# QCLovers/PyTDSCF

Hardware: NVIDIA B200
Metric: tdvp_sweeps_per_sec (higher is better)
Workload: dtype complex128

## Files before the change

pytdscf_b200/csrc/api.cu:

```cuda
#include <cstring>

#include "contract.cuh"

namespace tdvp {

int krylov_expm_exec(Handle* h, int kind, double scale_re, double scale_im, double thresh, int n_warmup,
                     int conserve_norm, const tdvp_heff_term* hterms, const tdvp_keff_term* kterms, int nterms,
                     int Dl, int d, int Dr, c128* psi, int* niter);
int lanczos_eigvec_exec(Handle* h, const tdvp_heff_term* hterms, int nterms, int Dl, int d, int Dr, c128* psi, int root,
                        double thresh, int* niter);
int inner_exec(Handle* h, long long n, const c128* bra, const c128* ket, int conj, c128* host_out);
int qr_shift_exec(Handle* h, int gauge, int Dl, int d, int Dr, const c128* psi, c128* site, c128* sigma);
int absorb_exec(Handle* h, int gauge, int Dl, int d, int Dr, int k, const c128* sigma, const c128* site, c128* out);
int qr_configure(Handle* h);
int svd_configure(Handle* h);

void set_error(Handle* h, const std::string& msg) {
  if (h) h->err = msg;
}

int cuda_fail(Handle* h, cudaError_t e, const char* what, const char* file, int line) {
  char buf[512];
  snprintf(buf, sizeof(buf), "CUDA error %d (%s) in %s at %s:%d", (int)e, cudaGetErrorString(e), what, file, line);
  set_error(h, buf);
  return (int)e > 0 ? (int)e : 1;
}

int ws_reserve(Handle* h, size_t bytes) {
  h->ws_top = 0;
  if (bytes <= h->ws_bytes) return 0;
  size_t want = bytes + bytes / 4 + (size_t(1) << 20);
  TDVP_CUDA(h, cudaStreamSynchronize(h->stream));
  if (h->side) TDVP_CUDA(h, cudaStreamSynchronize(h->side));
  if (h->ws) TDVP_CUDA(h, cudaFree(h->ws));
  h->ws = nullptr;
  h->ws_bytes = 0;
  void* p = nullptr;
  TDVP_CUDA(h, cudaMalloc(&p, want));
  h->ws = (unsigned char*)p;
  h->ws_bytes = want;
  return 0;
}

int ws_grow_preserve(Handle* h, size_t bytes) {
  if (bytes <= h->ws_bytes) return 0;
  void* p = nullptr;
  TDVP_CUDA(h, cudaMalloc(&p, bytes));
  if (h->ws) {
    cudaError_t e = cudaMemcpyAsync(p, h->ws, h->ws_top, cudaMemcpyDeviceToDevice, h->stream);
    if (e == cudaSuccess) e = cudaStreamSynchronize(h->stream);
    if (e != cudaSuccess) { cudaFree(p); return cuda_fail(h, e, "ws_grow_preserve copy", __FILE__, __LINE__); }
    TDVP_CUDA(h, cudaFree(h->ws));
  }
  h->ws = (unsigned char*)p;
  h->ws_bytes = bytes;
  return 0;
}

void* ws_alloc(Handle* h, size_t bytes) {
  const size_t b = align256(bytes);
  if (h->ws_top + b > h->ws_bytes) return nullptr;
  void* p = h->ws + h->ws_top;
  h->ws_top += b;
  return p;
}

}

using namespace tdvp;

struct tdvp_handle_s : public tdvp::Handle {};

#define H_CHECK(h)            \
  if (!(h)) return TDVP_ERR_ARG; \
  (h)->err.clear();

extern "C" {

int tdvp_abi_version(void) { return 2; }

unsigned long long tdvp_launch_count(void) { return tdvp::launch_count(); }

int tdvp_create(int device, void* cuda_stream, tdvp_handle_t* out) {
  if (!out) return TDVP_ERR_ARG;
  *out = nullptr;
  int ndev = 0;
  cudaError_t e = cudaGetDeviceCount(&ndev);
  if (e != cudaSuccess || ndev <= 0) return e != cudaSuccess ? (int)e : (int)cudaErrorNoDevice;
  if (device < 0 || device >= ndev) return TDVP_ERR_ARG;
  if ((e = cudaSetDevice(device)) != cudaSuccess) return (int)e;
  tdvp_handle_s* h = new tdvp_handle_s();
  h->device = device;
  h->stream = (cudaStream_t)cuda_stream;
  if ((e = cudaMalloc((void**)&h->d_scal, 4096 * sizeof(double))) != cudaSuccess) { delete h; return (int)e; }
  if ((e = cudaMallocHost((void**)&h->h_scal, 4096 * sizeof(double))) != cudaSuccess) { delete h; return (int)e; }
  if ((e = cudaMalloc((void**)&h->d_partial, 1024 * 64 * sizeof(double))) != cudaSuccess) { delete h; return (int)e; }
  if ((e = cudaMalloc((void**)&h->d_counter, 16 * sizeof(unsigned int))) != cudaSuccess) { delete h; return (int)e; }
  if ((e = cudaMalloc((void**)&h->d_splitk, tdvp::SPLITK_SCRATCH_ELEMS * sizeof(c128))) != cudaSuccess) { delete h; return (int)e; }
  if ((e = cudaMalloc((void**)&h->d_partial_side, 1024 * 64 * sizeof(double))) != cudaSuccess ||
      (e = cudaMalloc((void**)&h->d_counter_side, 16 * sizeof(unsigned int))) != cudaSuccess ||
      (e = cudaStreamCreateWithFlags(&h->side, cudaStreamNonBlocking)) != cudaSuccess ||
      (e = cudaEventCreateWithFlags(&h->ev_main, cudaEventDisableTiming)) != cudaSuccess ||
      (e = cudaEventCreateWithFlags(&h->ev_side, cudaEventDisableTiming)) != cudaSuccess) { tdvp_destroy(h); return (int)e; }
  cudaMemsetAsync(h->d_counter, 0, 16 * sizeof(unsigned int), h->stream);
  cudaMemsetAsync(h->d_counter_side, 0, 16 * sizeof(unsigned int), h->stream);
  cudaMemsetAsync(h->d_scal, 0, 4096 * sizeof(double), h->stream);
  memset(h->h_scal, 0, 4096 * sizeof(double));
  cudaDeviceGetAttribute(&h->num_sms, cudaDevAttrMultiProcessorCount, device);
  h->gemm.stream = h->stream;
  h->gemm.scratch = h->d_splitk;
  h->gemm.scratch_elems = tdvp::SPLITK_SCRATCH_ELEMS;
  h->gemm.num_sms = h->num_sms;
  h->gemm.sk_slots = h->num_sms;
  if ((e = cudaMalloc((void**)&h->gemm.sk_ws, sizeof(c128) * tdvp::STREAMK_TILE_ELEMS * (size_t)h->num_sms)) != cudaSuccess ||
      (e = cudaMalloc((void**)&h->gemm.sk_flags, sizeof(int) * (size_t)h->num_sms)) != cudaSuccess) { tdvp_destroy(h); return (int)e; }
  cudaMemsetAsync(h->gemm.sk_flags, 0, sizeof(int) * (size_t)h->num_sms, h->stream);
  int rc = 0;
  if ((e = tdvp::zgemm_configure_device(h->gemm)) != cudaSuccess) rc = (int)e;
  if (!rc) rc = tdvp::qr_configure(h);
  if (!rc) rc = tdvp::svd_configure(h);
  if (rc) { tdvp_destroy(h); return rc; }
  *out = h;
  return 0;
}

int tdvp_set_gemm_config(tdvp_handle_t h, int tile_cfg, int splitk, int c_stream) {
  if (!h || tile_cfg < 0 || tile_cfg > 5 || splitk < 0 || splitk > 16 || c_stream < 0 || c_stream > 2) return TDVP_ERR_ARG;
  h->gemm.force_cfg = tile_cfg;
  h->gemm.force_splitk = splitk;
  h->gemm.force_cstream = c_stream;
  return 0;
}

int tdvp_destroy(tdvp_handle_t h) {
  if (!h) return 0;
  cudaSetDevice(h->device);
  cudaStreamSynchronize(h->stream);
  if (h->ws) cudaFree(h->ws);
  if (h->d_scal) cudaFree(h->d_scal);
  if (h->h_scal) cudaFreeHost(h->h_scal);
  if (h->d_partial) cudaFree(h->d_partial);
  if (h->d_counter) cudaFree(h->d_counter);
  if (h->d_splitk) cudaFree(h->d_splitk);
  if (h->side) { cudaStreamSynchronize(h->side); cudaStreamDestroy(h->side); }
  if (h->ev_main) cudaEventDestroy(h->ev_main);
  if (h->ev_side) cudaEventDestroy(h->ev_side);
  if (h->d_partial_side) cudaFree(h->d_partial_side);
  if (h->d_counter_side) cudaFree(h->d_counter_side);
  if (h->gemm.sk_ws) cudaFree(h->gemm.sk_ws);
  if (h->gemm.sk_flags) cudaFree(h->gemm.sk_flags);
  delete h;
  return 0;
}

const char* tdvp_last_error(tdvp_handle_t h) { return h ? h->err.c_str() : "null handle"; }

int tdvp_get_stats(tdvp_handle_t h, unsigned long long* solves, unsigned long long* matvecs, double* flops) {
  if (!h) return TDVP_ERR_ARG;
  if (solves) *solves = h->krylov_solves;
  if (matvecs) *matvecs = h->krylov_matvecs;
  if (flops) *flops = h->heff_flops;
  return 0;
}

int tdvp_reset_stats(tdvp_handle_t h) {
  if (!h) return TDVP_ERR_ARG;
  h->krylov_solves = 0;
  h->krylov_matvecs = 0;
  h->heff_flops = 0.0;
  return 0;
}

int tdvp_gemm_profile(int enable, int reset, double* ms, double* flops, unsigned long long* launches) {
  tdvp::prof_collect(false);
  tdvp::prof_gemm_totals(ms, flops, launches);
  if (reset) tdvp::prof_collect(true);
  tdvp::prof_enable(enable != 0);
  return 0;
}

size_t tdvp_profile_json(char* out, size_t cap) {
  tdvp::prof_collect(false);
  return tdvp::prof_json(out, cap);
}

int tdvp_heff_apply(tdvp_handle_t h, const tdvp_heff_term* terms, int nterms, int Dl, int d, int Dr,
                    const tdvp_c128* psi, tdvp_c128* out) {
  H_CHECK(h);
  if (!terms || !psi || !out || Dl <= 0 || d <= 0 || Dr <= 0) { set_error(h, "heff_apply: bad argument"); return TDVP_ERR_ARG; }
  if (psi == out) { set_error(h, "heff_apply: out must not alias psi"); return TDVP_ERR_ARG; }
  TDVP_TRY(ws_reserve(h, sizeof(c128) * heff_ws_elems(terms, nterms, Dl, d, Dr)));
  return heff_apply_exec(h, terms, nterms, Dl, d, Dr, (const c128*)psi, (c128*)out);
}

int tdvp_keff_apply(tdvp_handle_t h, const tdvp_keff_term* terms, int nterms, int Dl, int Dr, const tdvp_c128* sigma,
                    tdvp_c128* out) {
  H_CHECK(h);
  if (!terms || !sigma || !out || Dl <= 0 || Dr <= 0) { set_error(h, "keff_apply: bad argument"); return TDVP_ERR_ARG; }
  if (sigma == out) { set_error(h, "keff_apply: out must not alias sigma"); return TDVP_ERR_ARG; }
  TDVP_TRY(ws_reserve(h, sizeof(c128) * keff_ws_elems(terms, nterms, Dl, Dr)));
  return keff_apply_exec(h, terms, nterms, Dl, Dr, (const c128*)sigma, (c128*)out);
}

int tdvp_env_update(tdvp_handle_t h, int gauge, int Dl, int d, int Dr, const tdvp_c128* bra, const tdvp_c128* ket,
                    const tdvp_c128* E, int w_in, const tdvp_c128* W, int w_kind, int w_out, tdvp_c128* out,
                    int accumulate) {
  H_CHECK(h);
  if (!bra || !ket || !out || Dl <= 0 || d <= 0 || Dr <= 0 || w_in <= 0 || w_out <= 0) { set_error(h, "env_update: bad argument"); return TDVP_ERR_ARG; }
  TDVP_TRY(ws_reserve(h, sizeof(c128) * env_ws_elems(Dl, d, Dr, w_in, w_out)));
  return env_update_exec(h, gauge, Dl, d, Dr, (const c128*)bra, (const c128*)ket, (const c128*)E, w_in, (const c128*)W,
                         w_kind, w_out, (c128*)out, accumulate != 0);
}

int tdvp_set_krylov_size(tdvp_handle_t hh, long long size) {
  Handle* h = reinterpret_cast<Handle*>(hh);
  if (!h || size < 0) return TDVP_ERR_ARG;
  h->krylov_size_override = size;
  return 0;
}

int tdvp_krylov_expm(tdvp_handle_t h, int kind, double scale_re, double scale_im, double thresh, int n_warmup,
                     int conserve_norm, const tdvp_heff_term* hterms, const tdvp_keff_term* kterms, int nterms, int Dl,
                     int d, int Dr, tdvp_c128* psi_inout, int* niter) {
  H_CHECK(h);
  if (!psi_inout || nterms <= 0 || Dl <= 0 || Dr <= 0 || (hterms && d <= 0)) { set_error(h, "krylov_expm: bad argument"); return TDVP_ERR_ARG; }
  return krylov_expm_exec(h, kind, scale_re, scale_im, thresh, n_warmup, conserve_norm, hterms, kterms, nterms, Dl, d, Dr,
                          (c128*)psi_inout, niter);
}

int tdvp_lanczos_eigvec(tdvp_handle_t h, const tdvp_heff_term* hterms, int nterms, int Dl, int d, int Dr,
                        tdvp_c128* psi_inout, int root, double thresh, int* niter) {
  H_CHECK(h);
  if (!hterms || !psi_inout || nterms <= 0 || Dl <= 0 || d <= 0 || Dr <= 0) { set_error(h, "lanczos_eigvec: bad argument"); return TDVP_ERR_ARG; }
  return lanczos_eigvec_exec(h, hterms, nterms, Dl, d, Dr, (c128*)psi_inout, root, thresh, niter);
}

int tdvp_qr_shift(tdvp_handle_t h, int gauge, int Dl, int d, int Dr, const tdvp_c128* psi, tdvp_c128* site,
                  tdvp_c128* sigma) {
  H_CHECK(h);
  if (!psi || !site || !sigma || Dl <= 0 || d <= 0 || Dr <= 0) { set_error(h, "qr_shift: bad argument"); return TDVP_ERR_ARG; }
  return qr_shift_exec(h, gauge, Dl, d, Dr, (const c128*)psi, (c128*)site, (c128*)sigma);
}

int tdvp_absorb(tdvp_handle_t h, int gauge, int Dl, int d, int Dr, int k, const tdvp_c128* sigma, const tdvp_c128* site,
                tdvp_c128* out) {
  H_CHECK(h);
  if (!sigma || !site || !out || Dl <= 0 || d <= 0 || Dr <= 0 || k <= 0) { set_error(h, "absorb: bad argument"); return TDVP_ERR_ARG; }
  return absorb_exec(h, gauge, Dl, d, Dr, k, (const c128*)sigma, (const c128*)site, (c128*)out);
}

int tdvp_inner(tdvp_handle_t h, long long n, const tdvp_c128* bra, const tdvp_c128* ket, int conj, tdvp_c128* host_out) {
  H_CHECK(h);
  if (!bra || !ket || !host_out || n <= 0) { set_error(h, "inner: bad argument"); return TDVP_ERR_ARG; }
  return inner_exec(h, n, (const c128*)bra, (const c128*)ket, conj, (c128*)host_out);
}

int tdvp_overlap_site(tdvp_handle_t h, int Dlb, int Dlk, int d, int Drb, int Drk, const tdvp_c128* bra,
                      const tdvp_c128* ket, const tdvp_c128* block, int conj_bra, tdvp_c128* out) {
  H_CHECK(h);
  if (!bra || !ket || !block || !out) { set_error(h, "overlap_site: bad argument"); return TDVP_ERR_ARG; }
  TDVP_TRY(ws_reserve(h, sizeof(c128) * ((size_t)Dlb * d * Drk + 64)));
  return overlap_site_exec(h, Dlb, Dlk, d, Drb, Drk, (const c128*)bra, (const c128*)ket, (const c128*)block, conj_bra,
                           (c128*)out);
}

int tdvp_zgemm(tdvp_handle_t h, int transA, int transB, int M, int N, int K, double alpha_re, double alpha_im,
               const tdvp_c128* A, int lda, const tdvp_c128* B, int ldb, double beta_re, double beta_im, tdvp_c128* C,
               int ldc) {
  H_CHECK(h);
  if (!A || !B || !C || M < 0 || N < 0 || K < 0 || transA < 0 || transA > 2 || transB < 0 || transB > 2) {
    set_error(h, "zgemm: bad argument");
    return TDVP_ERR_ARG;
  }
  GemmDesc g = gemm_rowmajor(M, N, K, (const c128*)A, lda, transA != 0, transA == 2, (const c128*)B, ldb, transB != 0,
                             (c128*)C, ldc, c128{alpha_re, alpha_im}, c128{beta_re, beta_im});
  g.b_conj = transB == 2 ? 1 : 0;
  return gemm(h, g);
}

}
```

pytdscf_b200/csrc/build.py:

```python
from __future__ import annotations

import hashlib
import os
import subprocess
import sys

HERE = os.path.dirname(os.path.abspath(__file__))
PKG = os.path.dirname(HERE)
SOURCES = ["api.cu", "zgemm.cu", "zgemm_tma.cu", "contract.cu", "krylov.cu", "qr.cu", "svd.cu"]
HEADERS = ["common.cuh", "handle.cuh", "contract.cuh", "zgemm_plan.h", os.path.join("..", "..", "include", "tdvp_b200.h")]
OUT = os.path.join(PKG, "libtdvp_b200.so")
NVCC_FLAGS = [
    "-gencode", "arch=compute_100a,code=sm_100a",
    "-O3", "-lineinfo", "-std=c++17",
    "-Xcompiler", "-fPIC",
]


def _digest() -> str:
    h = hashlib.sha256()
    for f in SOURCES + HEADERS:
        p = os.path.join(HERE, f)
        if os.path.exists(p):
            h.update(open(p, "rb").read())
    h.update(" ".join(NVCC_FLAGS).encode())
    return h.hexdigest()


def build(force: bool = False, verbose: bool = True) -> str:
    stamp = OUT + ".sha256"
    dig = _digest()
    if not force and os.path.exists(OUT) and os.path.exists(stamp) and open(stamp).read().strip() == dig:
        return OUT
    nvcc = os.environ.get("NVCC", "nvcc")
    objs = []
    os.makedirs(os.path.join(HERE, "_obj"), exist_ok=True)
    procs = []
    for src in SOURCES:
        sp = os.path.join(HERE, src)
        if not os.path.exists(sp):
            continue
        obj = os.path.join(HERE, "_obj", src.replace(".cu", ".o"))
        objs.append(obj)
        cmd = [nvcc, *NVCC_FLAGS, "-c", sp, "-o", obj]
        if verbose:
            print("[build]", " ".join(cmd), flush=True)
        procs.append((src, subprocess.Popen(cmd, stdout=subprocess.PIPE, stderr=subprocess.STDOUT, text=True)))
    failed = False
    for src, p in procs:
        out, _ = p.communicate()
        if p.returncode != 0:
            failed = True
            print(f"[build] {src} FAILED:\n{out}", file=sys.stderr)
        elif out.strip() and verbose:
            print(out)
    if failed:
        raise RuntimeError("nvcc failed")
    cmd = [nvcc, "-gencode", "arch=compute_100a,code=sm_100a", "-shared", "-o", OUT, *objs, "-lcudart"]
    if verbose:
        print("[build]", " ".join(cmd), flush=True)
    subprocess.check_call(cmd)
    with open(stamp, "w") as f:
        f.write(dig)
    return OUT


if __name__ == "__main__":
    print(build(force="--force" in sys.argv))
```

pytdscf_b200/csrc/handle.cuh:

```cuda
#pragma once
#include "common.cuh"

#include <vector>

namespace tdvp {

struct Handle {
  int device = 0;
  cudaStream_t stream = nullptr;
  std::string err;
  unsigned char* ws = nullptr;
  size_t ws_bytes = 0;
  size_t ws_top = 0;
  double* d_scal = nullptr;
  double* h_scal = nullptr;
  double* d_partial = nullptr;
  unsigned int* d_counter = nullptr;
  c128* d_splitk = nullptr;
  cudaStream_t side = nullptr;
  cudaEvent_t ev_main = nullptr, ev_side = nullptr;
  double* d_partial_side = nullptr;
  unsigned int* d_counter_side = nullptr;
  GemmCtx gemm;
  int num_sms = 148;
  int qr_max_cluster = 0;
  int svd_max_blocks = 0;
  int svd_blocked_max_blocks = 0;
  unsigned long long krylov_matvecs = 0;
  unsigned long long krylov_solves = 0;
  long long krylov_size_override = 0;
  double heff_flops = 0.0;
};

int ws_reserve(Handle* h, size_t bytes);
int ws_grow_preserve(Handle* h, size_t bytes);
void* ws_alloc(Handle* h, size_t bytes);
inline void ws_reset(Handle* h) { h->ws_top = 0; }
inline size_t align256(size_t b) { return (b + 255) & ~size_t(255); }

}
```

pytdscf_b200/csrc/qr.cu:

```cuda
#include <cooperative_groups.h>

#include "contract.cuh"

namespace cg = cooperative_groups;

namespace tdvp {

namespace {

constexpr int NB = 32;
constexpr int SLAB_ROWS = 256;
constexpr int PT = 256;
constexpr int PTY = PT / 32;

struct PanelArgs {
  c128* A; int lda; int m; int n; int j0; int jb;
  double* tau;
  c128* Vall;
  c128* Tall;
  double* gpart;
  double* zpart;
  int rows_per_cta;
  c128* gslab;
  int dbg;
};

__device__ __forceinline__ double dlapy3(double x, double y, double z) {
  const double w = fmax(fabs(x), fmax(fabs(y), fabs(z)));
  if (w == 0.0) return 0.0;
  const double a = x / w, b = y / w, c = z / w;
  return w * sqrt(a * a + b * b + c * c);
}

__global__ void __launch_bounds__(PT, 1) k_qr_panel(PanelArgs p) {
  extern __shared__ __align__(16) unsigned char smraw[];
  c128* S = p.gslab ? p.gslab + (size_t)blockIdx.x * p.rows_per_cta * NB : reinterpret_cast<c128*>(smraw);
  __shared__ c128 red[PTY][NB];
  __shared__ c128 gtot[NB];
  __shared__ c128 rowc[NB];
  __shared__ c128 wv[NB];
  __shared__ double s_tau[2], s_scal[2], s_beta;
  cg::grid_group grid = cg::this_grid();
  const int tx = threadIdx.x, ty = threadIdx.y;
  const int G = gridDim.x, b = blockIdx.x;
  const int jb = p.jb, j0 = p.j0;
  const int r0 = j0 + b * p.rows_per_cta;
  int nrow = p.m - r0;
  if (nrow > p.rows_per_cta) nrow = p.rows_per_cta;
  if (nrow < 0) nrow = 0;

  for (int i = ty; i < nrow; i += PTY) {
    if (tx < jb) S[i * NB + tx] = p.A[(long long)(r0 + i) * p.lda + j0 + tx];
    else S[i * NB + tx] = {0.0, 0.0};
  }
  __syncthreads();

  for (int c = 0; c < jb; ++c) {
    const int grow = j0 + c;
    double* gp = p.gpart + (size_t)(c & 1) * G * (4 * NB);
    c128 acc = {0.0, 0.0};
    if (tx >= c && tx < jb) {
      for (int i = ty; i < nrow; i += PTY) {
        if (r0 + i > grow) {
          const c128 x = S[i * NB + c], y = S[i * NB + tx];
          acc.x += x.x * y.x + x.y * y.y;
          acc.y += x.x * y.y - x.y * y.x;
        }
      }
    }
    red[ty][tx] = acc;
    __syncthreads();
    if (ty == 0) {
      c128 t = {0.0, 0.0};
#pragma unroll
      for (int q = 0; q < PTY; ++q) { t.x += red[q][tx].x; t.y += red[q][tx].y; }
      gp[(size_t)b * (4 * NB) + 2 * tx] = t.x;
      gp[(size_t)b * (4 * NB) + 2 * tx + 1] = t.y;
      if (grow >= r0 && grow < r0 + nrow) {
        const c128 v = S[(grow - r0) * NB + tx];
        gp[2 * NB + 2 * tx] = v.x;
        gp[2 * NB + 2 * tx + 1] = v.y;
      }
    }
    __threadfence();
    if (G > 1) grid.sync(); else __syncthreads();
    if (ty == 0) {
      c128 t = {0.0, 0.0};
      for (int q = 0; q < G; ++q) {
        t.x += __ldcg(&gp[(size_t)q * (4 * NB) + 2 * tx]);
        t.y += __ldcg(&gp[(size_t)q * (4 * NB) + 2 * tx + 1]);
      }
      gtot[tx] = t;
      rowc[tx] = {__ldcg(&gp[2 * NB + 2 * tx]), __ldcg(&gp[2 * NB + 2 * tx + 1])};
    }
    __syncthreads();
    if (tx == 0 && ty == 0) {
      const bool tiny_tail = gtot[c].x < 1.0e-200;
      const double xnorm = tiny_tail ? 0.0 : sqrt(gtot[c].x);
      const double alphr = rowc[c].x, alphi = rowc[c].y;
      if (xnorm == 0.0 && alphi == 0.0) {
        s_tau[0] = 0.0; s_tau[1] = 0.0; s_scal[0] = 1.0; s_scal[1] = 0.0; s_beta = alphr;
      } else if (tiny_tail) {
        const double beta = (alphr >= 0.0) ? -hypot(alphr, alphi) : hypot(alphr, alphi);
        s_tau[0] = (beta - alphr) / beta;
        s_tau[1] = -alphi / beta;
        s_scal[0] = 0.0; s_scal[1] = 0.0;
        s_beta = beta;
      } else {
        double beta = dlapy3(alphr, alphi, xnorm);
        beta = (alphr >= 0.0) ? -beta : beta;
        s_tau[0] = (beta - alphr) / beta;
        s_tau[1] = -alphi / beta;
        const double dr = alphr - beta, di = alphi;
        const double den = dr * dr + di * di;
        s_scal[0] = dr / den; s_scal[1] = -di / den;
        s_beta = beta;
      }
      if (b == 0) { p.tau[2 * (j0 + c)] = s_tau[0]; p.tau[2 * (j0 + c) + 1] = s_tau[1]; }
    }
    __syncthreads();
    const c128 tau = {s_tau[0], s_tau[1]};
    const c128 sc = {s_scal[0], s_scal[1]};
    const bool trivial = (tau.x == 0.0 && tau.y == 0.0);
    if (ty == 0 && tx > c && tx < jb) {
      const c128 cs = {sc.x, -sc.y};
      wv[tx] = cadd(rowc[tx], cmul(cs, gtot[tx]));
    }
    __syncthreads();
    if (!trivial) {
      const c128 ctau = {tau.x, -tau.y};
      for (int i = ty; i < nrow; i += PTY) {
        const int gr = r0 + i;
        if (gr < grow) continue;
        c128 v;
        if (gr == grow) v = {1.0, 0.0};
        else v = cmul(S[i * NB + c], sc);
        if (tx > c && tx < jb) {
          const c128 f = cmul(ctau, cmul(v, wv[tx]));
          S[i * NB + tx].x -= f.x;
          S[i * NB + tx].y -= f.y;
        }
        __syncwarp();
        if (tx == c) S[i * NB + c] = (gr == grow) ? c128{s_beta, 0.0} : v;
      }
    }
    __syncthreads();
  }

  for (int i = ty; i < nrow; i += PTY) {
    const int gr = r0 + i;
    if (tx < jb) {
      const c128 a = S[i * NB + tx];
      p.A[(long long)gr * p.lda + j0 + tx] = a;
      c128 v;
      const int dcol = gr - j0;
      if (tx < dcol) v = a;
      else if (tx == dcol) v = {1.0, 0.0};
      else v = {0.0, 0.0};
      p.Vall[(long long)gr * p.lda + j0 + tx] = v;
      S[i * NB + tx] = v;
    }
  }
  __syncthreads();
  for (int a = ty; a < jb; a += PTY) {
    c128 z = {0.0, 0.0};
    if (tx < jb && a < tx) {
      for (int i = 0; i < nrow; ++i) {
        const c128 x = S[i * NB + a], y = S[i * NB + tx];
        z.x += x.x * y.x + x.y * y.y;
        z.y += x.x * y.y - x.y * y.x;
      }
    }
    p.zpart[((size_t)b * NB + a) * NB * 2 + 2 * tx] = z.x;
    p.zpart[((size_t)b * NB + a) * NB * 2 + 2 * tx + 1] = z.y;
  }
  __threadfence();
  if (G > 1) grid.sync(); else __syncthreads();
  if (b != 0) return;
  c128* Z = S;
  c128* T = S + NB * NB;
  for (int a = ty; a < NB; a += PTY) {
    c128 z = {0.0, 0.0};
    for (int q = 0; q < G; ++q) {
      z.x += __ldcg(&p.zpart[((size_t)q * NB + a) * NB * 2 + 2 * tx]);
      z.y += __ldcg(&p.zpart[((size_t)q * NB + a) * NB * 2 + 2 * tx + 1]);
    }
    Z[a * NB + tx] = z;
    T[a * NB + tx] = {0.0, 0.0};
  }
  __syncthreads();
  for (int c = 0; c < jb; ++c) {
    const c128 tau = {__ldcg(&p.tau[2 * (j0 + c)]), __ldcg(&p.tau[2 * (j0 + c) + 1])};
    if (ty == 0 && tx < c) {
      c128 s = {0.0, 0.0};
      for (int q = tx; q < c; ++q) s = cadd(s, cmul(T[tx * NB + q], Z[q * NB + c]));
      const c128 r = cmul(tau, s);
      T[tx * NB + c] = {-r.x, -r.y};
    }
    if (ty == 0 && tx == c) T[c * NB + c] = tau;
    __syncthreads();
  }
  c128* Tout = p.Tall + (size_t)(j0 / NB) * NB * NB;
  for (int a = ty; a < NB; a += PTY) Tout[a * NB + tx] = T[a * NB + tx];
}


constexpr int CT = 512;
constexpr int CTY = CT / 32;
constexpr int MAXG = 16;
constexpr int CL_ROWS = 256;

__device__ __forceinline__ unsigned qr_smem_u32(const void* p) { return (unsigned)__cvta_generic_to_shared(p); }
__device__ __forceinline__ unsigned qr_mapa(unsigned local, int cta) {
  unsigned r;
  asm volatile("mapa.shared::cluster.u32 %0, %1, %2;\n" : "=r"(r) : "r"(local), "r"(cta));
  return r;
}
__device__ __forceinline__ void qr_push(unsigned remote_addr, c128 v, unsigned remote_bar) {
  asm volatile("st.async.weak.shared::cluster.mbarrier::complete_tx::bytes.v2.f64 [%0], {%1, %2}, [%3];\n" ::"r"(remote_addr),
               "d"(v.x), "d"(v.y), "r"(remote_bar)
               : "memory");
}
__device__ __forceinline__ bool qr_try_wait(unsigned bar, unsigned parity) {
  unsigned ok;
  asm volatile(
      "{\n"
      ".reg .pred p;\n"
      "mbarrier.try_wait.parity.shared::cta.b64 p, [%1], %2;\n"
      "selp.b32 %0, 1, 0, p;\n"
      "}\n"
      : "=r"(ok)
      : "r"(bar), "r"(parity)
      : "memory");
  return ok != 0;
}

__device__ __forceinline__ void zlarfg_scalars(double alphr, double alphi, double g2, c128& tau, c128& sc, double& hbeta) {
  const bool tiny_tail = g2 < 1.0e-200;
  if (tiny_tail && alphi == 0.0) { tau = {0.0, 0.0}; sc = {1.0, 0.0}; hbeta = alphr; return; }
  if (tiny_tail) {
    const double beta = (alphr >= 0.0) ? -hypot(alphr, alphi) : hypot(alphr, alphi);
    tau = {(beta - alphr) / beta, -alphi / beta};
    sc = {0.0, 0.0};
    hbeta = beta;
    return;
  }
  double beta;
  if (g2 < 1.0e280 && fabs(alphr) < 1.0e140 && fabs(alphi) < 1.0e140) beta = sqrt(alphr * alphr + alphi * alphi + g2);
  else beta = dlapy3(alphr, alphi, sqrt(g2));
  beta = (alphr >= 0.0) ? -beta : beta;
  const double rb = 1.0 / beta;
  tau = {(beta - alphr) * rb, -alphi * rb};
  const double dr = alphr - beta, di = alphi;
  const double rd = 1.0 / (dr * dr + di * di);
  sc = {dr * rd, -di * rd};
  hbeta = beta;
}

__global__ void __launch_bounds__(CT, 1) k_qr_panel_cluster(PanelArgs p) {
  extern __shared__ __align__(16) unsigned char smraw[];
  c128* S = reinterpret_cast<c128*>(smraw);
  __shared__ c128 red[CTY][NB + 1];
  __shared__ __align__(16) c128 inbox[2][MAXG + 1][NB];
  __shared__ __align__(8) unsigned long long mbar[2];
  __shared__ c128 gtot[NB], rowc[NB], rowstage[NB];
  __shared__ double s_zl[5];
  cg::cluster_group cluster = cg::this_cluster();
  const int tx = threadIdx.x, ty = threadIdx.y;
  const int G = gridDim.x, b = blockIdx.x;
  const int jb = p.jb, j0 = p.j0;
  const int r0 = j0 + b * p.rows_per_cta;
  int nrow = p.m - r0;
  if (nrow > p.rows_per_cta) nrow = p.rows_per_cta;
  if (nrow < 0) nrow = 0;

  if (tx == 0 && ty == 0) {
    asm volatile("mbarrier.init.shared::cta.b64 [%0], 1;\n" ::"r"(qr_smem_u32(&mbar[0])) : "memory");
    asm volatile("mbarrier.init.shared::cta.b64 [%0], 1;\n" ::"r"(qr_smem_u32(&mbar[1])) : "memory");
    asm volatile("fence.mbarrier_init.release.cluster;\n" ::: "memory");
  }
  for (int i = ty; i < nrow; i += CTY) {
    if (tx < jb) S[i * NB + tx] = p.A[(long long)(r0 + i) * p.lda + j0 + tx];
    else S[i * NB + tx] = {0.0, 0.0};
  }
  __syncthreads();
  cluster.sync();

  constexpr int MAXPER = (CL_ROWS + CTY - 1) / CTY;
  c128 mine[MAXPER];
#pragma unroll
  for (int k = 0; k < MAXPER; ++k) {
    const int i = ty + CTY * k;
    mine[k] = (i < nrow) ? S[i * NB + tx] : c128{0.0, 0.0};
  }
  c128 acc = {0.0, 0.0};
#pragma unroll
  for (int k = 0; k < MAXPER; ++k) {
    const int i = ty + CTY * k;
    const double xr = __shfl_sync(0xffffffffu, mine[k].x, 0), xi = __shfl_sync(0xffffffffu, mine[k].y, 0);
    if (i < nrow && r0 + i > j0 && tx < jb) {
      acc.x += xr * mine[k].x + xi * mine[k].y;
      acc.y += xr * mine[k].y - xi * mine[k].x;
    }
    if (i < nrow && r0 + i == j0) rowstage[tx] = mine[k];
  }
  for (int c = 0; c < ((p.dbg & 1) ? 0 : jb); ++c) {
    const int grow = j0 + c;
    const int buf = c & 1;
    const unsigned parity = (unsigned)(c >> 1) & 1u;
    const int owner = c / p.rows_per_cta;
    red[ty][tx] = acc;
    __syncthreads();
    {
      const int half = tx >> 4, q = tx & 15, col = ty + CTY * half;
      c128 t = red[q][col];
#pragma unroll
      for (int o = 8; o > 0; o >>= 1) {
        t.x += __shfl_xor_sync(0xffffffffu, t.x, o);
        t.y += __shfl_xor_sync(0xffffffffu, t.y, o);
      }
      const unsigned bar_local = qr_smem_u32(&mbar[buf]);
      if (q < G) qr_push(qr_mapa(qr_smem_u32(&inbox[buf][b][col]), q), t, qr_mapa(bar_local, q));
      if (b == owner && ty < G) qr_push(qr_mapa(qr_smem_u32(&inbox[buf][MAXG][tx]), ty), rowstage[tx], qr_mapa(bar_local, ty));
    }
    if (ty == 0) {
      const unsigned bar = qr_smem_u32(&mbar[buf]);
      if (tx == 0) {
        const unsigned bytes = (unsigned)((G + 1) * NB * sizeof(c128));
        asm volatile("mbarrier.arrive.expect_tx.shared::cta.b64 _, [%0], %1;\n" ::"r"(bar), "r"(bytes) : "memory");
      }
      __syncwarp();
      while (!qr_try_wait(bar, parity)) {
      }
      c128 t = {0.0, 0.0};
#pragma unroll
      for (int q = 0; q < MAXG; ++q) {
        if (q < G) { const c128 v = inbox[buf][q][tx]; t.x += v.x; t.y += v.y; }
      }
      const c128 rc = inbox[buf][MAXG][tx];
      gtot[tx] = t;
      rowc[tx] = rc;
      const double g2 = __shfl_sync(0xffffffffu, t.x, c);
      const double alphr = __shfl_sync(0xffffffffu, rc.x, c), alphi = __shfl_sync(0xffffffffu, rc.y, c);
      c128 tau_, sc_;
      double hb_;
      zlarfg_scalars(alphr, alphi, g2, tau_, sc_, hb_);
      if (tx == 0) {
        s_zl[0] = tau_.x; s_zl[1] = tau_.y; s_zl[2] = sc_.x; s_zl[3] = sc_.y; s_zl[4] = hb_;
        if (b == 0) { p.tau[2 * (j0 + c)] = tau_.x; p.tau[2 * (j0 + c) + 1] = tau_.y; }
      }
    }
    __syncthreads();
    const c128 tau = {s_zl[0], s_zl[1]}, sc = {s_zl[2], s_zl[3]};
    const double hbeta = s_zl[4];
    const bool trivial = (tau.x == 0.0 && tau.y == 0.0);
    c128 yj = {0.0, 0.0}, ydj = {0.0, 0.0};
    if (tx > c && tx < jb) {
      const c128 cs = {sc.x, -sc.y};
      const c128 wv = cadd(rowc[tx], cmul(cs, gtot[tx]));
      const c128 ctau = {tau.x, -tau.y};
      ydj = cmul(ctau, wv);
      yj = cmul(sc, ydj);
    }
    acc = {0.0, 0.0};
    const int cn = (c + 1 < NB) ? c + 1 : c;
#pragma unroll
    for (int k = 0; k < MAXPER; ++k) {
      const int i = ty + CTY * k;
      const int gr = r0 + i;
      if (i >= nrow || gr < grow) continue;
      if (!trivial) {
        const double xr = __shfl_sync(0xffffffffu, mine[k].x, c), xi = __shfl_sync(0xffffffffu, mine[k].y, c);
        const c128 x = {xr, xi};
        if (tx > c && tx < jb) {
          const c128 f = (gr == grow) ? ydj : cmul(x, yj);
          mine[k].x -= f.x;
          mine[k].y -= f.y;
        }
        if (tx == c) mine[k] = (gr == grow) ? c128{hbeta, 0.0} : cmul(x, sc);
      }
      const double nr = __shfl_sync(0xffffffffu, mine[k].x, cn);
      const double ni = __shfl_sync(0xffffffffu, mine[k].y, cn);
      if (gr > grow + 1 && tx > c && tx < jb) {
        acc.x += nr * mine[k].x + ni * mine[k].y;
        acc.y += nr * mine[k].y - ni * mine[k].x;
      }
      if (gr == grow + 1) rowstage[tx] = mine[k];
    }
  }
#pragma unroll
  for (int k = 0; k < MAXPER; ++k) {
    const int i = ty + CTY * k;
    if (i < nrow) S[i * NB + tx] = mine[k];
  }
  __syncthreads();

  for (int i = ty; i < nrow; i += CTY) {
    const int gr = r0 + i;
    if (tx < jb) {
      const c128 a = S[i * NB + tx];
      p.A[(long long)gr * p.lda + j0 + tx] = a;
      c128 v;
      const int dcol = gr - j0;
      if (tx < dcol) v = a;
      else if (tx == dcol) v = {1.0, 0.0};
      else v = {0.0, 0.0};
      p.Vall[(long long)gr * p.lda + j0 + tx] = v;
      S[i * NB + tx] = v;
    }
  }
  __syncthreads();
  for (int a = ty; a < NB; a += CTY) {
    c128 z = {0.0, 0.0};
    if (tx < jb && a < tx) {
      for (int i = 0; i < nrow; ++i) {
        const c128 x = S[i * NB + a], y = S[i * NB + tx];
        z.x += x.x * y.x + x.y * y.y;
        z.y += x.x * y.y - x.y * y.x;
      }
    }
    p.zpart[((size_t)b * NB + a) * NB * 2 + 2 * tx] = z.x;
    p.zpart[((size_t)b * NB + a) * NB * 2 + 2 * tx + 1] = z.y;
  }
  __threadfence();
  cluster.sync();
  if (b != 0) return;
  c128* Z = S;
  c128* Tt = S + NB * NB;
  __shared__ c128 taus[NB];
  for (int a = ty; a < NB; a += CTY) {
    c128 z = {0.0, 0.0};
    for (int q = 0; q < G; ++q) {
      z.x += __ldcg(&p.zpart[((size_t)q * NB + a) * NB * 2 + 2 * tx]);
      z.y += __ldcg(&p.zpart[((size_t)q * NB + a) * NB * 2 + 2 * tx + 1]);
    }
    Z[a * NB + tx] = z;
    Tt[a * NB + tx] = {0.0, 0.0};
    if (a == 0) taus[tx] = (tx < jb) ? c128{__ldcg(&p.tau[2 * (j0 + tx)]), __ldcg(&p.tau[2 * (j0 + tx) + 1])} : c128{0.0, 0.0};
  }
  __syncthreads();
  if (ty == 0 && !(p.dbg & 2)) {
    const int r = tx;
    if (r < jb) {
      Tt[r * NB + r] = taus[r];
      for (int c = r + 1; c < jb; ++c) {
        c128 s0 = {0.0, 0.0}, s1 = {0.0, 0.0};
        int q = r;
        for (; q + 1 < c; q += 2) {
          const c128 a0 = Tt[q * NB + r], z0 = Z[q * NB + c];
          const c128 a1 = Tt[(q + 1) * NB + r], z1 = Z[(q + 1) * NB + c];
          s0.x += a0.x * z0.x - a0.y * z0.y; s0.y += a0.x * z0.y + a0.y * z0.x;
          s1.x += a1.x * z1.x - a1.y * z1.y; s1.y += a1.x * z1.y + a1.y * z1.x;
        }
        if (q < c) {
          const c128 a0 = Tt[q * NB + r], z0 = Z[q * NB + c];
          s0.x += a0.x * z0.x - a0.y * z0.y; s0.y += a0.x * z0.y + a0.y * z0.x;
        }
        const c128 rr = cmul(taus[c], cadd(s0, s1));
        Tt[c * NB + r] = {-rr.x, -rr.y};
      }
    }
  }
  __syncthreads();
  c128* Tout = p.Tall + (size_t)(j0 / NB) * NB * NB;
  for (int a = ty; a < NB; a += CTY) Tout[a * NB + tx] = Tt[tx * NB + a];
}

__global__ void k_set_identity(c128* Q, int m, int n, int ld) {
  const long long tot = (long long)m * n;
  for (long long e = blockIdx.x * (long long)blockDim.x + threadIdx.x; e < tot; e += (long long)gridDim.x * blockDim.x) {
    const int i = e / n, j = e % n;
    Q[(long long)i * ld + j] = {i == j ? 1.0 : 0.0, 0.0};
  }
}

__global__ void k_extract_r(const c128* A, int lda, int k, int n, c128* R, int ldr, int transpose) {
  const long long tot = (long long)k * n;
  for (long long e = blockIdx.x * (long long)blockDim.x + threadIdx.x; e < tot; e += (long long)gridDim.x * blockDim.x) {
    const int i = e / n, j = e % n;
    const c128 v = (j >= i) ? A[(long long)i * lda + j] : c128{0.0, 0.0};
    if (transpose) R[(long long)j * ldr + i] = v; else R[(long long)i * ldr + j] = v;
  }
}

GemmDesc vhc_desc(int jb, int nc, int mp, const c128* V, long long ldv, const c128* C, long long ldc, c128* W, const char* tag) {
  GemmDesc g;
  g.M = nc; g.N = jb; g.K = mp;
  g.A = C; g.a_m_inner = 1; g.a_m1 = 1; g.a_m0 = 0; g.a_k = ldc; g.a_conj = 0;
  g.B = V; g.b_n_inner = 1; g.b_n1 = 1; g.b_n0 = 0; g.b_k = ldv; g.b_conj = 1;
  g.C = W; g.c_m_inner = 1; g.c_m1 = 1; g.c_m0 = 0; g.c_n = nc;
  g.tag = tag;
  return g;
}

int lq(Handle* h, const char* what) {
  count_launch();
  cudaError_t e = cudaGetLastError();
  if (e != cudaSuccess) return cuda_fail(h, e, what, __FILE__, __LINE__);
  return 0;
}

}

constexpr int QR_MAX_SMS = 256;

size_t qr_ws_elems(int m, int n) {
  const size_t np = (n + NB - 1) / NB;
  return 3 * (size_t)m * n + (size_t)(m + QR_MAX_SMS) * NB + np * NB * NB + 2 * (size_t)NB * n + 4096 + (size_t)QR_MAX_SMS * NB * NB + QR_MAX_SMS * 4 * NB;
}

int qr_configure(Handle* h) {
  TDVP_CUDA(h, cudaFuncSetAttribute(k_qr_panel, cudaFuncAttributeMaxDynamicSharedMemorySize, SLAB_ROWS * NB * (int)sizeof(c128)));
  TDVP_CUDA(h, cudaFuncSetAttribute(k_qr_panel_cluster, cudaFuncAttributeMaxDynamicSharedMemorySize, CL_ROWS * NB * (int)sizeof(c128)));
  TDVP_CUDA(h, cudaFuncSetAttribute(k_qr_panel_cluster, cudaFuncAttributeNonPortableClusterSizeAllowed, 1));
  h->qr_max_cluster = 0;
  for (int cs : {16, 8, 4, 2, 1}) {
    cudaLaunchConfig_t cfg = {};
    cfg.gridDim = dim3(cs);
    cfg.blockDim = dim3(32, CTY);
    cfg.dynamicSmemBytes = CL_ROWS * NB * sizeof(c128);
    cudaLaunchAttribute at[1];
    at[0].id = cudaLaunchAttributeClusterDimension;
    at[0].val.clusterDim.x = cs; at[0].val.clusterDim.y = 1; at[0].val.clusterDim.z = 1;
    cfg.attrs = at; cfg.numAttrs = 1;
    int nclusters = 0;
    if (cudaOccupancyMaxActiveClusters(&nclusters, k_qr_panel_cluster, &cfg) == cudaSuccess && nclusters >= 1) { h->qr_max_cluster = cs; break; }
  }
  cudaGetLastError();
  if (h->num_sms > QR_MAX_SMS) { set_error(h, "qr: device has more SMs than the workspace bound"); return TDVP_ERR_UNSUPPORTED; }
  return 0;
}

int qr_factor(Handle* h, c128* A, int m, int n, int lda, c128* Q, int ldq) {
  if (m < n) { set_error(h, "qr_factor: needs m >= n"); return TDVP_ERR_SHAPE; }
  const int max_coop = h->num_sms;
  const int max_cluster = h->qr_max_cluster;
  const int qr_dbg = 0;
  const int np = (n + NB - 1) / NB;
  c128* Vall = (c128*)ws_alloc(h, sizeof(c128) * (size_t)m * lda);
  c128* Tall = (c128*)ws_alloc(h, sizeof(c128) * (size_t)np * NB * NB);
  c128* W = (c128*)ws_alloc(h, sizeof(c128) * (size_t)NB * n);
  c128* W2 = (c128*)ws_alloc(h, sizeof(c128) * (size_t)NB * n);
  double* tau = (double*)ws_alloc(h, sizeof(double) * 2 * (size_t)n);
  double* gpart = (double*)ws_alloc(h, sizeof(double) * 2 * (size_t)max_coop * 4 * NB);
  double* zpart = (double*)ws_alloc(h, sizeof(double) * 2 * (size_t)max_coop * NB * NB);
  c128* gslab = (m > max_coop * SLAB_ROWS) ? (c128*)ws_alloc(h, sizeof(c128) * (size_t)(m + max_coop) * NB) : nullptr;
  if (!Vall || !Tall || !W || !W2 || !tau || !gpart || !zpart || (m > max_coop * SLAB_ROWS && !gslab)) {
    set_error(h, "qr_factor: workspace");
    return TDVP_ERR_ARG;
  }
  TDVP_CUDA(h, cudaMemsetAsync(Vall, 0, sizeof(c128) * (size_t)m * lda, h->stream));
  const c128 one = {1.0, 0.0}, zero = {0.0, 0.0}, mone = {-1.0, 0.0};

  for (int pnl = 0; pnl < np; ++pnl) {
    const int j0 = pnl * NB;
    const int jb = (n - j0) < NB ? (n - j0) : NB;
    const int mp = m - j0;
    cudaError_t e;
    if (max_cluster >= 1 && mp <= max_cluster * CL_ROWS) {
      int G = 1;
      constexpr int rows_target = 64;
      while (G < max_cluster && (mp + G - 1) / G > rows_target) G *= 2;
      while ((mp + G - 1) / G > CL_ROWS) G *= 2;
      const int rpc = (mp + G - 1) / G;
      PanelArgs pa{A, lda, m, n, j0, jb, tau, Vall, Tall, gpart, zpart, rpc, nullptr, qr_dbg};
      cudaLaunchConfig_t cfg = {};
      cfg.gridDim = dim3(G);
      cfg.blockDim = dim3(32, CTY);
      cfg.dynamicSmemBytes = sizeof(c128) * (size_t)(rpc > 2 * NB ? rpc : 2 * NB) * NB;
      cfg.stream = h->stream;
      cudaLaunchAttribute at[1];
      at[0].id = cudaLaunchAttributeClusterDimension;
      at[0].val.clusterDim.x = G; at[0].val.clusterDim.y = 1; at[0].val.clusterDim.z = 1;
      cfg.attrs = at; cfg.numAttrs = 1;
      { ProfScope _ps(h->stream, "qr.k_qr_panel_cluster"); e = cudaLaunchKernelEx(&cfg, k_qr_panel_cluster, pa); }
      count_launch();
      if (e != cudaSuccess) return cuda_fail(h, e, "cudaLaunchKernelEx(k_qr_panel_cluster)", __FILE__, __LINE__);
    } else {
      int rpc = SLAB_ROWS;
      int G = (mp + rpc - 1) / rpc;
      const bool global_slabs = G > max_coop;
      if (global_slabs) G = max_coop;
      if (G < 1) G = 1;
      rpc = (mp + G - 1) / G;
      PanelArgs pa{A, lda, m, n, j0, jb, tau, Vall, Tall, gpart, zpart, rpc, global_slabs ? gslab : nullptr, qr_dbg};
      void* args[] = {&pa};
      const size_t smem = global_slabs ? 0 : sizeof(c128) * (size_t)(rpc > 2 * NB ? rpc : 2 * NB) * NB;
      { ProfScope _ps(h->stream, "qr.k_qr_panel"); e = cudaLaunchCooperativeKernel((void*)k_qr_panel, dim3(G), dim3(32, PTY), args, smem, h->stream); }
      count_launch();
      if (e != cudaSuccess) return cuda_fail(h, e, "cudaLaunchCooperativeKernel(k_qr_panel)", __FILE__, __LINE__);
    }
    const int nc = n - j0 - jb;
    if (nc > 0) {
      c128* Vp = Vall + (long long)j0 * lda + j0;
      c128* C = A + (long long)j0 * lda + j0 + jb;
      c128* T = Tall + (size_t)pnl * NB * NB;
      TDVP_TRY(gemm(h, vhc_desc(jb, nc, mp, Vp, lda, C, lda, W, "qr.VhC")));
      TDVP_TRY(gemm(h, tagged(gemm_rowmajor(jb, nc, jb, T, NB, true, true, W, nc, false, W2, nc, one, zero), "qr.TW")));
      TDVP_TRY(gemm(h, tagged(gemm_rowmajor(mp, nc, jb, Vp, lda, false, false, W2, nc, false, C, lda, mone, one), "qr.VW")));
    }
  }
  { ProfScope _ps(h->stream, "qr.k_set_identity"); k_set_identity<<<148 * 2, 256, 0, h->stream>>>(Q, m, n, ldq); }
  TDVP_TRY(lq(h, "k_set_identity"));
  for (int pnl = np - 1; pnl >= 0; --pnl) {
    const int j0 = pnl * NB;
    const int jb = (n - j0) < NB ? (n - j0) : NB;
    const int mp = m - j0;
    const int nc = n - j0;
    c128* Vp = Vall + (long long)j0 * lda + j0;
    c128* C = Q + (long long)j0 * ldq + j0;
    c128* T = Tall + (size_t)pnl * NB * NB;
    TDVP_TRY(gemm(h, vhc_desc(jb, nc, mp, Vp, lda, C, ldq, W, "ungqr.VhC")));
    TDVP_TRY(gemm(h, tagged(gemm_rowmajor(jb, nc, jb, T, NB, false, false, W, nc, false, W2, nc, one, zero), "ungqr.TW")));
    TDVP_TRY(gemm(h, tagged(gemm_rowmajor(mp, nc, jb, Vp, lda, false, false, W2, nc, false, C, ldq, mone, one), "ungqr.VW")));
  }
  return 0;
}

int qr_shift_exec(Handle* h, int gauge, int Dl, int d, int Dr, const c128* psi, c128* site, c128* sigma) {
  const long long N = (long long)Dl * d * Dr;
  const int m = (gauge == TDVP_GAUGE_A) ? Dl * d : Dr * d;
  const int n = (gauge == TDVP_GAUGE_A) ? Dr : Dl;
  if (m < n) { set_error(h, "qr_shift: matricisation has fewer rows than columns (bond dimension rule violated)"); return TDVP_ERR_SHAPE; }
  TDVP_TRY(ws_reserve(h, sizeof(c128) * (qr_ws_elems(m, n) + 2 * (size_t)N) + 4096));
  c128* Awork = (c128*)ws_alloc(h, sizeof(c128) * (size_t)N);
  if (!Awork) { set_error(h, "qr_shift: workspace"); return TDVP_ERR_ARG; }
  if (gauge == TDVP_GAUGE_A) {
    TDVP_CUDA(h, cudaMemcpyAsync(Awork, psi, sizeof(c128) * N, cudaMemcpyDeviceToDevice, h->stream));
    TDVP_TRY(qr_factor(h, Awork, m, n, n, site, n));
    { ProfScope _ps(h->stream, "qr.k_extract_r"); k_extract_r<<<64, 256, 0, h->stream>>>(Awork, n, n, n, sigma, n, 0); }
    TDVP_TRY(lq(h, "k_extract_r"));
  } else if (gauge == TDVP_GAUGE_B) {
    c128* Qt = (c128*)ws_alloc(h, sizeof(c128) * (size_t)N);
    if (!Qt) { set_error(h, "qr_shift: workspace"); return TDVP_ERR_ARG; }
    TDVP_TRY(permute_site(h, psi, Awork, Dl, d, Dr));
    TDVP_TRY(qr_factor(h, Awork, m, n, n, Qt, n));
    TDVP_TRY(permute_site(h, Qt, site, Dr, d, n));
    { ProfScope _ps(h->stream, "qr.k_extract_r"); k_extract_r<<<64, 256, 0, h->stream>>>(Awork, n, n, n, sigma, n, 1); }
    TDVP_TRY(lq(h, "k_extract_r"));
  } else {
    set_error(h, "qr_shift: bad gauge");
    return TDVP_ERR_ARG;
  }
  return 0;
}

int absorb_exec(Handle* h, int gauge, int Dl, int d, int Dr, int k, const c128* sigma, const c128* site, c128* out) {
  TDVP_TRY(ws_reserve(h, 4096));
  if (gauge == TDVP_GAUGE_A) {
    return gemm(h, tagged(gemm_rowmajor(k, d * Dr, Dl, sigma, Dl, false, false, site, (long long)d * Dr, false, out, (long long)d * Dr), "absorb"));
  } else if (gauge == TDVP_GAUGE_B) {
    return gemm(h, tagged(gemm_rowmajor(Dl * d, k, Dr, site, Dr, false, false, sigma, k, false, out, k), "absorb"));
  }
  set_error(h, "absorb: bad gauge");
  return TDVP_ERR_ARG;
}

}
```

Measured before the change: 0.5812.

## Add look-ahead QR that overlaps the next panel with the trailing update

The blocked Householder QR now first updates only the next panel's columns. It then factors that panel on the main stream while the rest of the trailing-matrix update runs on a new high-priority side stream, with events ordering the two. A planner checks that the split GEMMs choose the same kernel configuration as the unsplit one and falls back to a single update otherwise. The side-stream GEMMs get an SM budget reduced by the panel's cluster size and no stream-K workspace. The aim is to take the serial panel factorization off the critical path, at the cost of extra GEMM launches and event synchronization.

```diff
diff --git a/pytdscf_b200/csrc/api.cu b/pytdscf_b200/csrc/api.cu
--- a/pytdscf_b200/csrc/api.cu
+++ b/pytdscf_b200/csrc/api.cu
@@ -102,6 +102,13 @@
       (e = cudaStreamCreateWithFlags(&h->side, cudaStreamNonBlocking)) != cudaSuccess ||
       (e = cudaEventCreateWithFlags(&h->ev_main, cudaEventDisableTiming)) != cudaSuccess ||
       (e = cudaEventCreateWithFlags(&h->ev_side, cudaEventDisableTiming)) != cudaSuccess) { tdvp_destroy(h); return (int)e; }
+  {
+    int lo = 0, hi = 0;
+    if ((e = cudaDeviceGetStreamPriorityRange(&lo, &hi)) != cudaSuccess ||
+        (e = cudaStreamCreateWithPriority(&h->qr_side, cudaStreamNonBlocking, hi)) != cudaSuccess ||
+        (e = cudaEventCreateWithFlags(&h->qr_ev[0], cudaEventDisableTiming)) != cudaSuccess ||
+        (e = cudaEventCreateWithFlags(&h->qr_ev[1], cudaEventDisableTiming)) != cudaSuccess) { tdvp_destroy(h); return (int)e; }
+  }
   cudaMemsetAsync(h->d_counter, 0, 16 * sizeof(unsigned int), h->stream);
   cudaMemsetAsync(h->d_counter_side, 0, 16 * sizeof(unsigned int), h->stream);
   cudaMemsetAsync(h->d_scal, 0, 4096 * sizeof(double), h->stream);
@@ -145,6 +152,9 @@
   if (h->side) { cudaStreamSynchronize(h->side); cudaStreamDestroy(h->side); }
   if (h->ev_main) cudaEventDestroy(h->ev_main);
   if (h->ev_side) cudaEventDestroy(h->ev_side);
+  if (h->qr_side) { cudaStreamSynchronize(h->qr_side); cudaStreamDestroy(h->qr_side); }
+  for (cudaEvent_t ev : h->qr_ev)
+    if (ev) cudaEventDestroy(ev);
   if (h->d_partial_side) cudaFree(h->d_partial_side);
   if (h->d_counter_side) cudaFree(h->d_counter_side);
   if (h->gemm.sk_ws) cudaFree(h->gemm.sk_ws);
diff --git a/pytdscf_b200/csrc/build.py b/pytdscf_b200/csrc/build.py
--- a/pytdscf_b200/csrc/build.py
+++ b/pytdscf_b200/csrc/build.py
@@ -8,7 +8,7 @@
 HERE = os.path.dirname(os.path.abspath(__file__))
 PKG = os.path.dirname(HERE)
 SOURCES = ["api.cu", "zgemm.cu", "zgemm_tma.cu", "contract.cu", "krylov.cu", "qr.cu", "svd.cu"]
-HEADERS = ["common.cuh", "handle.cuh", "contract.cuh", "zgemm_plan.h", os.path.join("..", "..", "include", "tdvp_b200.h")]
+HEADERS = ["common.cuh", "handle.cuh", "contract.cuh", "zgemm_plan.h", "qr_plan.h", os.path.join("..", "..", "include", "tdvp_b200.h")]
 OUT = os.path.join(PKG, "libtdvp_b200.so")
 NVCC_FLAGS = [
     "-gencode", "arch=compute_100a,code=sm_100a",
diff --git a/pytdscf_b200/csrc/handle.cuh b/pytdscf_b200/csrc/handle.cuh
--- a/pytdscf_b200/csrc/handle.cuh
+++ b/pytdscf_b200/csrc/handle.cuh
@@ -21,6 +21,8 @@
   cudaEvent_t ev_main = nullptr, ev_side = nullptr;
   double* d_partial_side = nullptr;
   unsigned int* d_counter_side = nullptr;
+  cudaStream_t qr_side = nullptr;
+  cudaEvent_t qr_ev[2] = {nullptr, nullptr};
   GemmCtx gemm;
   int num_sms = 148;
   int qr_max_cluster = 0;
diff --git a/pytdscf_b200/csrc/qr.cu b/pytdscf_b200/csrc/qr.cu
--- a/pytdscf_b200/csrc/qr.cu
+++ b/pytdscf_b200/csrc/qr.cu
@@ -1,6 +1,7 @@
 #include <cooperative_groups.h>
 
 #include "contract.cuh"
+#include "qr_plan.h"
 
 namespace cg = cooperative_groups;
 
@@ -8,7 +9,7 @@
 
 namespace {
 
-constexpr int NB = 32;
+constexpr int NB = QR_NB;
 constexpr int SLAB_ROWS = 256;
 constexpr int PT = 256;
 constexpr int PTY = PT / 32;
@@ -208,7 +209,7 @@
 constexpr int CT = 512;
 constexpr int CTY = CT / 32;
 constexpr int MAXG = 16;
-constexpr int CL_ROWS = 256;
+constexpr int CL_ROWS = QR_CL_ROWS;
 
 __device__ __forceinline__ unsigned qr_smem_u32(const void* p) { return (unsigned)__cvta_generic_to_shared(p); }
 __device__ __forceinline__ unsigned qr_mapa(unsigned local, int cta) {
@@ -483,16 +484,6 @@
   }
 }
 
-GemmDesc vhc_desc(int jb, int nc, int mp, const c128* V, long long ldv, const c128* C, long long ldc, c128* W, const char* tag) {
-  GemmDesc g;
-  g.M = nc; g.N = jb; g.K = mp;
-  g.A = C; g.a_m_inner = 1; g.a_m1 = 1; g.a_m0 = 0; g.a_k = ldc; g.a_conj = 0;
-  g.B = V; g.b_n_inner = 1; g.b_n1 = 1; g.b_n0 = 0; g.b_k = ldv; g.b_conj = 1;
-  g.C = W; g.c_m_inner = 1; g.c_m1 = 1; g.c_m0 = 0; g.c_n = nc;
-  g.tag = tag;
-  return g;
-}
-
 int lq(Handle* h, const char* what) {
   count_launch();
   cudaError_t e = cudaGetLastError();
@@ -552,31 +543,29 @@
   TDVP_CUDA(h, cudaMemsetAsync(Vall, 0, sizeof(c128) * (size_t)m * lda, h->stream));
   const c128 one = {1.0, 0.0}, zero = {0.0, 0.0}, mone = {-1.0, 0.0};
 
-  for (int pnl = 0; pnl < np; ++pnl) {
-    const int j0 = pnl * NB;
-    const int jb = (n - j0) < NB ? (n - j0) : NB;
-    const int mp = m - j0;
+  static const char* const tags[2][3] = {{"qr.VhC", "qr.TW", "qr.VW"}, {"qr.la.VhC", "qr.la.TW", "qr.la.VW"}};
+  const cudaStream_t streams[2] = {h->stream, h->qr_side};
+  for (const QrOp& op : plan_qr(m, n, lda, h->gemm, max_cluster)) {
+    const cudaStream_t st = streams[op.stream];
+    const int j0 = op.j0, jb = op.jb, mp = m - j0;
     cudaError_t e;
-    if (max_cluster >= 1 && mp <= max_cluster * CL_ROWS) {
-      int G = 1;
-      constexpr int rows_target = 64;
-      while (G < max_cluster && (mp + G - 1) / G > rows_target) G *= 2;
-      while ((mp + G - 1) / G > CL_ROWS) G *= 2;
+    if (op.kind == QR_PANEL && op.cluster > 0) {
+      const int G = op.cluster;
       const int rpc = (mp + G - 1) / G;
       PanelArgs pa{A, lda, m, n, j0, jb, tau, Vall, Tall, gpart, zpart, rpc, nullptr, qr_dbg};
       cudaLaunchConfig_t cfg = {};
       cfg.gridDim = dim3(G);
       cfg.blockDim = dim3(32, CTY);
       cfg.dynamicSmemBytes = sizeof(c128) * (size_t)(rpc > 2 * NB ? rpc : 2 * NB) * NB;
-      cfg.stream = h->stream;
+      cfg.stream = st;
       cudaLaunchAttribute at[1];
       at[0].id = cudaLaunchAttributeClusterDimension;
       at[0].val.clusterDim.x = G; at[0].val.clusterDim.y = 1; at[0].val.clusterDim.z = 1;
       cfg.attrs = at; cfg.numAttrs = 1;
-      { ProfScope _ps(h->stream, "qr.k_qr_panel_cluster"); e = cudaLaunchKernelEx(&cfg, k_qr_panel_cluster, pa); }
+      { ProfScope _ps(st, "qr.k_qr_panel_cluster"); e = cudaLaunchKernelEx(&cfg, k_qr_panel_cluster, pa); }
       count_launch();
       if (e != cudaSuccess) return cuda_fail(h, e, "cudaLaunchKernelEx(k_qr_panel_cluster)", __FILE__, __LINE__);
-    } else {
+    } else if (op.kind == QR_PANEL) {
       int rpc = SLAB_ROWS;
       int G = (mp + rpc - 1) / rpc;
       const bool global_slabs = G > max_coop;
@@ -586,18 +575,23 @@
       PanelArgs pa{A, lda, m, n, j0, jb, tau, Vall, Tall, gpart, zpart, rpc, global_slabs ? gslab : nullptr, qr_dbg};
       void* args[] = {&pa};
       const size_t smem = global_slabs ? 0 : sizeof(c128) * (size_t)(rpc > 2 * NB ? rpc : 2 * NB) * NB;
-      { ProfScope _ps(h->stream, "qr.k_qr_panel"); e = cudaLaunchCooperativeKernel((void*)k_qr_panel, dim3(G), dim3(32, PTY), args, smem, h->stream); }
+      { ProfScope _ps(st, "qr.k_qr_panel"); e = cudaLaunchCooperativeKernel((void*)k_qr_panel, dim3(G), dim3(32, PTY), args, smem, st); }
       count_launch();
       if (e != cudaSuccess) return cuda_fail(h, e, "cudaLaunchCooperativeKernel(k_qr_panel)", __FILE__, __LINE__);
-    }
-    const int nc = n - j0 - jb;
-    if (nc > 0) {
-      c128* Vp = Vall + (long long)j0 * lda + j0;
-      c128* C = A + (long long)j0 * lda + j0 + jb;
-      c128* T = Tall + (size_t)pnl * NB * NB;
-      TDVP_TRY(gemm(h, vhc_desc(jb, nc, mp, Vp, lda, C, lda, W, "qr.VhC")));
-      TDVP_TRY(gemm(h, tagged(gemm_rowmajor(jb, nc, jb, T, NB, true, true, W, nc, false, W2, nc, one, zero), "qr.TW")));
-      TDVP_TRY(gemm(h, tagged(gemm_rowmajor(mp, nc, jb, Vp, lda, false, false, W2, nc, false, C, lda, mone, one), "qr.VW")));
+    } else if (op.kind == QR_UPDATE) {
+      GemmDesc g[3];
+      qr_update_descs(g, jb, op.c1 - op.c0, mp, Vall + (long long)j0 * lda + j0, lda, Tall + (size_t)(j0 / NB) * NB * NB,
+                      A + (long long)j0 * lda + op.c0, lda, W, W2, true, tags[op.overlap]);
+      for (int k = 0; k < 3; ++k) {
+        if (!op.split) { TDVP_TRY(gemm(h, g[k])); continue; }
+        const GemmCtx fc = forced_ctx(h->gemm, op.force_cfg[k], op.force_splitk[k]);
+        e = zgemm_auto(g[k], op.overlap ? overlap_ctx(fc, op.cluster, st) : fc);
+        if (e != cudaSuccess) return cuda_fail(h, e, g[k].tag, __FILE__, __LINE__);
+      }
+    } else if (op.kind == QR_RECORD) {
+      TDVP_CUDA(h, cudaEventRecord(h->qr_ev[op.event], st));
+    } else {
+      TDVP_CUDA(h, cudaStreamWaitEvent(st, h->qr_ev[op.event], 0));
     }
   }
   { ProfScope _ps(h->stream, "qr.k_set_identity"); k_set_identity<<<148 * 2, 256, 0, h->stream>>>(Q, m, n, ldq); }
diff --git a/pytdscf_b200/csrc/qr_plan.h b/pytdscf_b200/csrc/qr_plan.h
--- /dev/null
+++ b/pytdscf_b200/csrc/qr_plan.h
@@ -0,0 +1,138 @@
+#pragma once
+#include <vector>
+
+#include "zgemm_plan.h"
+
+namespace tdvp {
+
+constexpr int QR_NB = 32;
+constexpr int QR_CL_ROWS = 256;
+
+enum QrOpKind : int {
+  QR_PANEL = 0,
+  QR_UPDATE = 1,
+  QR_RECORD = 2,
+  QR_WAIT = 3,
+};
+enum QrStream : int { QR_MAIN = 0, QR_SIDE = 1 };
+
+struct QrOp {
+  int kind = QR_PANEL;
+  int stream = QR_MAIN;
+  int j0 = 0, jb = 0;
+  int c0 = 0, c1 = 0;
+  int cluster = 0;
+  int event = 0;
+  int split = 0, overlap = 0;
+  int force_cfg[3] = {0, 0, 0}, force_splitk[3] = {0, 0, 0};
+};
+
+inline int qr_panel_cluster(int mp, int max_cluster) {
+  if (max_cluster < 1 || mp > max_cluster * QR_CL_ROWS) return 0;
+  int G = 1;
+  constexpr int rows_target = 64;
+  while (G < max_cluster && (mp + G - 1) / G > rows_target) G *= 2;
+  while ((mp + G - 1) / G > QR_CL_ROWS) G *= 2;
+  return G;
+}
+
+inline GemmDesc vhc_desc(int jb, int nc, int mp, const c128* V, long long ldv, const c128* C, long long ldc, c128* W, const char* tag) {
+  GemmDesc g;
+  g.M = nc; g.N = jb; g.K = mp;
+  g.A = C; g.a_m_inner = 1; g.a_m1 = 1; g.a_m0 = 0; g.a_k = ldc; g.a_conj = 0;
+  g.B = V; g.b_n_inner = 1; g.b_n1 = 1; g.b_n0 = 0; g.b_k = ldv; g.b_conj = 1;
+  g.C = W; g.c_m_inner = 1; g.c_m1 = 1; g.c_m0 = 0; g.c_n = nc;
+  g.tag = tag;
+  return g;
+}
+
+inline void qr_update_descs(GemmDesc out[3], int jb, int nc, int mp, const c128* V, long long ldv, const c128* T, c128* C,
+                            long long ldc, c128* W, c128* W2, bool adjoint, const char* const tags[3]) {
+  const c128 one = {1.0, 0.0}, zero = {0.0, 0.0}, mone = {-1.0, 0.0};
+  out[0] = vhc_desc(jb, nc, mp, V, ldv, C, ldc, W, tags[0]);
+  out[1] = tagged(gemm_rowmajor(jb, nc, jb, T, QR_NB, adjoint, adjoint, W, nc, false, W2, nc, one, zero), tags[1]);
+  out[2] = tagged(gemm_rowmajor(mp, nc, jb, V, ldv, false, false, W2, nc, false, C, ldc, mone, one), tags[2]);
+}
+
+inline GemmCtx forced_ctx(const GemmCtx& ctx, int force_cfg, int force_splitk) {
+  GemmCtx c = ctx;
+  c.force_cfg = force_cfg;
+  c.force_splitk = force_splitk;
+  return c;
+}
+inline GemmCtx overlap_ctx(const GemmCtx& ctx, int cluster, cudaStream_t stream) {
+  GemmCtx c = ctx;
+  c.stream = stream;
+  c.sk_ws = nullptr;
+  c.sk_flags = nullptr;
+  c.num_sms = ctx.num_sms - cluster > 1 ? ctx.num_sms - cluster : 1;
+  return c;
+}
+
+inline std::vector<QrOp> plan_qr(int m, int n, int lda, const GemmCtx& ctx, int max_cluster) {
+  static const char* const no_tags[3] = {"", "", ""};
+  const c128* base = reinterpret_cast<const c128*>((uintptr_t)1 << 36);
+  c128* fake = const_cast<c128*>(base);
+  auto descs = [&](GemmDesc out[3], int j0, int jb, int c0, int c1) {
+    qr_update_descs(out, jb, c1 - c0, m - j0, base + (long long)j0 * lda + j0, lda, base, fake + (long long)j0 * lda + c0, lda,
+                    fake, fake, true, no_tags);
+  };
+  auto same = [](const GemmPlan& a, const GemmPlan& b) {
+    return a.kernel == b.kernel && a.S == b.S && a.k_chunk == b.k_chunk && a.reduce == b.reduce && a.streamk == 0 && b.streamk == 0;
+  };
+  std::vector<QrOp> ops;
+  const int np = (n + QR_NB - 1) / QR_NB;
+  auto width = [&](int j0) { return (n - j0) < QR_NB ? (n - j0) : QR_NB; };
+  auto push = [&](int kind, int st, int j0, int ev) {
+    QrOp o;
+    o.kind = kind; o.stream = st; o.j0 = j0; o.event = ev;
+    if (kind == QR_PANEL) { o.jb = width(j0); o.cluster = qr_panel_cluster(m - j0, max_cluster); }
+    ops.push_back(o);
+  };
+  bool factored = false;
+  for (int p = 0; p < np; ++p) {
+    const int j0 = p * QR_NB, jb = width(j0);
+    if (!factored) push(QR_PANEL, QR_MAIN, j0, 0);
+    factored = false;
+    const int c0 = j0 + jb;
+    if (c0 >= n) break;
+    const int c1 = c0 + width(c0);
+    const int G = qr_panel_cluster(m - c0, max_cluster);
+    QrOp u;
+    u.kind = QR_UPDATE; u.j0 = j0; u.jb = jb; u.c0 = c0; u.c1 = n;
+    bool split = G > 0 && c1 < n && ctx.force_cfg == 0 && ctx.force_splitk == 0;
+    if (split) {
+      GemmDesc whole[3], next[3], rest[3];
+      descs(whole, j0, jb, c0, n);
+      descs(next, j0, jb, c0, c1);
+      descs(rest, j0, jb, c1, n);
+      for (int g = 0; g < 3 && split; ++g) {
+        const GemmPlan pw = plan_gemm(whole[g], ctx);
+        const int cfg = (pw.kernel == GEMM_TMA_WIDE || pw.kernel == GEMM_TMA_TALL) ? 5 : pw.kernel;
+        const int sk = pw.S > 1 ? pw.S : 1;
+        const GemmCtx fc = forced_ctx(ctx, cfg, sk);
+        split = same(pw, plan_gemm(next[g], fc)) && same(pw, plan_gemm(rest[g], overlap_ctx(fc, G, ctx.stream)));
+        u.force_cfg[g] = cfg;
+        u.force_splitk[g] = sk;
+      }
+    }
+    if (!split) {
+      ops.push_back(u);
+      continue;
+    }
+    u.split = 1;
+    u.c1 = c1;
+    ops.push_back(u);
+    push(QR_RECORD, QR_MAIN, 0, 0);
+    push(QR_PANEL, QR_MAIN, c0, 0);
+    push(QR_WAIT, QR_SIDE, 0, 0);
+    u.c0 = c1; u.c1 = n; u.overlap = 1; u.cluster = G; u.stream = QR_SIDE;
+    ops.push_back(u);
+    push(QR_RECORD, QR_SIDE, 0, 1);
+    push(QR_WAIT, QR_MAIN, 0, 1);
+    factored = true;
+  }
+  return ops;
+}
+
+}
```

Result: no change. 0.5828, median of 6 (+0.3%).
